# cmpute/d3d

Measured on AMD Instinct MI355X. Metric: voxelize_mpoints_per_s, higher is better.
Workload: dtype f32; 1 GPU; config2: 1000000 LiDAR-like points, KITTI range, 0.1 m voxels (704x800x40), dense+MEAN, max 32 pts/voxel; points_per_gpu=1000000, parallelism=1 GPU

## Files before the change

### d3d_amd/csrc/voxel.hip

```cpp
#include "common.hpp"
#include <stdlib.h>
#include <limits.h>
#include <algorithm>
#include <utility>

namespace {

typedef unsigned long long u64;

constexpr u64 kEmpty = ~0ull;
constexpr uint32_t kInf = 0xffffffffu;
constexpr uint32_t kSingleVoxel = 0xfffffffeu;
constexpr uint32_t kNoVoxel = 0xffffffffu;
constexpr uint32_t kNoSlot = 0xffffffffu;
constexpr uint32_t kNoBase = 0xffffffffu;
constexpr int kReduceSum = 4;
constexpr int kSweepTile = 1024;
constexpr int kFlagTile = 256 * 64;


__device__ __forceinline__ u64 mix64(u64 h)
{
    h ^= h >> 33; h *= 0xff51afd7ed558ccdull;
    h ^= h >> 33; h *= 0xc4ceb9fe1a85ec53ull;
// ... 1951 lines not shown
            const typename E::type e = bent[pos[r]];
            key_in[r] = E::key(e);
            idx[r] = E::idx(e);
        }
    });
    if constexpr (STAGE) {
        static_for<ITEMS>([&](auto R) {
            constexpr int r = decltype(R)::value;
            row[r] = *reinterpret_cast<const v4f *>(&points4[idx[r]]);
        });
    }
    lds_barrier();
    D3D_PHASE(0, 1);
#ifdef D3D_PHASE_CLOCKS
    asm volatile("s_waitcnt vmcnt(0)" ::: "memory");
    D3D_PHASE(0, 8);
#endif
    static_for<ITEMS>([&](auto R) {
        constexpr int r = decltype(R)::value;
        const uint32_t q = threadIdx.x + r * kBucketThreads;
        if (q < m) {
            const KT key = (KT)key_in[r];
            uint32_t s = (Key::bin_hash(key_in[r]) >> hshift) & (T - 1);
            for (;;) {
                const KT old = atomicCAS(&tkey[s], kFree, key);
                if (old == kFree || old == key) break;
                s = (s + 1) & (T - 1);
            }
            slot[r] = s;
            arr[r] = atomicAdd(&tcnt[s], 1u);
            atomicMin(&tfirst[s], idx[r]);
        }
    });
    lds_barrier();
    D3D_PHASE(0, 2);
    records(std::false_type{});
    early_publish();
    lds_barrier();
    D3D_PHASE(0, 3);
    static_for<ITEMS>([&](auto R) {
        constexpr int r = decltype(R)::value;
        const uint32_t q = threadIdx.x + r * kBucketThreads;
        if (q < m) seg[(tcnt[slot[r]] >> 16) + arr[r]] = idx[r];
    });
    lds_barrier();
    D3D_PHASE(0, 4);
    v4f over_pre = {0.f, 0.f, 0.f, 0.f};
    if constexpr (ROWS) overflow_first(seg, over_pre);
    static_for<ITEMS>([&](auto R) {
        constexpr int r = decltype(R)::value;
        const uint32_t q = threadIdx.x + r * kBucketThreads;
        if (q < m) {
            const uint32_t s = slot[r], cb = tcnt[s], cnt = cb & 0xffffu, base = cb >> 16, me = idx[r];
            uint32_t rank = 0, k = 0;
            const uint32_t *sg = seg + base;
            const bool need = (STAGE || LISTS) ? cnt > 1 : cnt > P;
            for (; need && k + 8 <= cnt && rank < P; k += 8)
                rank += (sg[k] < me) + (sg[k + 1] < me) + (sg[k + 2] < me) + (sg[k + 3] < me) + (sg[k + 4] < me) + (sg[k + 5] < me) +
                        (sg[k + 6] < me) + (sg[k + 7] < me);
            for (; need && k < cnt && rank < P; k++) rank += sg[k] < me;
            if constexpr (STAGE) { if (rank < P) *reinterpret_cast<v4f *>(&staged[bb + base + rank]) = row[r]; }
            if constexpr (LISTS) {
                if (rank < P && (rank > 0 || !ROWS)) sorted_out[bb + base + rank] = me;
                if (unsorted_out && cnt > P) unsorted_out[bb + base + arr[r]] = me;
            }
            if (trimmed && rank >= P) trimmed[me] = 1;
            if (precpos) precpos[pos[r]] = tfirst[s];
            if (pfirst_out) {
                const uint32_t pf = (P > 0 && rank >= P) ? kInf : tfirst[s];
                if (!table || pf != me) pfirst_out[me] = pf;
            }
        }
    });
    D3D_PHASE(0, 5);
    reduce_overflow(seg, std::false_type{}, ROWS ? &over_pre : (const v4f *)nullptr);
    D3D_PHASE(0, 6);
}

struct EarlyNote {
    const u64 *tot = nullptr;
    uint32_t pairs = 0, max_voxels = 0;
    int64_t aux = 0;
    int64_t *counts = nullptr, *host = nullptr;
};

__global__ __launch_bounds__(1024) void k_first_count(const uint32_t *__restrict__ firstmap, uint32_t *fwpre, uint32_t *bsumF,
                                                      uint32_t *clear_word = nullptr ,
                                                      ZeroFill zf = ZeroFill(), EarlyNote en = EarlyNote())
{
    if (zero_fill_role(zf)) return;
    if (en.tot && blockIdx.x == 0 && threadIdx.x < kWave) {
        u64 v = 0;
        for (uint32_t t = threadIdx.x; t < en.pairs; t += kWave) v += en.tot[16 * t];
        v = wave_sum_u64(v);
        if (threadIdx.x == 0) {
            en.counts[D3D_COUNT_VOXELS] = (int64_t)(v < (u64)en.max_voxels ? v : (u64)en.max_voxels);
            en.counts[D3D_COUNT_AUX] = en.aux;
            notify_host(en.counts, en.host);
        }
    }
    if (clear_word && blockIdx.x == 0 && threadIdx.x == 0) *clear_word = 0;
    __shared__ u64 smem[1024 / kWave];
    __shared__ uint32_t wcnt[256];
    const int lane = threadIdx.x & (kWave - 1), w = threadIdx.x >> 6;
    const uint32_t *src = firstmap + ((size_t)blockIdx.x * 256 + w * 16) * 64 + lane;
    uint32_t e[16];
#pragma unroll
    for (int j = 0; j < 16; j++) e[j] = src[(size_t)j * 64];
#pragma unroll
    for (int j = 0; j < 16; j++) {
        const unsigned long long bal = __ballot(e[j] != kInf);
        if (lane == j) wcnt[w * 16 + j] = (uint32_t)__popcll(bal);
    }
    __syncthreads();
    u64 tot;
    const u64 ex = block_excl_scan_u64<1024>(threadIdx.x < 256 ? (u64)wcnt[threadIdx.x] : 0ull, &tot, smem);
    if (threadIdx.x < 256) fwpre[(size_t)blockIdx.x * 256 + threadIdx.x] = (uint32_t)ex;
    if (threadIdx.x == 0) bsumF[blockIdx.x] = (uint32_t)tot;
}

template <class Key, bool AGG4>
__device__ __forceinline__ uint32_t meta_first_lane(const Key &kf, int64_t i, uint32_t e, uint32_t vid, const uint4 *__restrict__ vrec,
                                                    uint32_t max_voxels, uint4 *__restrict__ vinfo, const float4 *__restrict__ staged,
                                                    uint32_t P, int reduction, int64_t *coords, int32_t *npoints, unsigned char *pmask,
                                                    float4 *agg, const BinnedExtras &x, const float *__restrict__ points, int c)
{
    uint32_t kept = 0, myvid = kNoVoxel;
    if (e != kInf && vid < max_voxels) {
        myvid = vid;
        if (x.first_out) x.first_out[vid] = x.index_offset + i;
        uint4 rec;
        if (e != kSingleVoxel) rec = vrec[e];
        else {
            const float *src = points + i * c;
            const float v3[3] = {src[0], src[1], src[2]};
            u64 key = 0;
            uint32_t st = 0;
            (void)kf.make(v3, key, st);
            rec = make_uint4((uint32_t)key, (uint32_t)(key >> 32), 0u, 1u);
        }
        const uint4 vi = rec;
        if (vinfo) vinfo[vid] = vi;
        if (x.count_out) x.count_out[vid] = (int32_t)vi.w;
        kept = vi.w < x.npoints_clamp ? vi.w : x.npoints_clamp;
        meta_voxel<Key, AGG4>(kf, (int64_t)vid, vi, staged, P, reduction, coords, npoints, x.voff, pmask, agg, nullptr, nullptr,
                              x.keys_out, x.npoints_clamp, x.has_coord_sub ? x.coord_sub : (const long long *)nullptr);
    }
    if (x.vidof) x.vidof[i] = myvid;
    return kept;
}

template <class Key, bool AGG4>
__global__ __launch_bounds__(256) void k_meta_first(Key kf, int64_t npad, const uint32_t *__restrict__ firstmap,
                                                    const uint32_t *__restrict__ fwpre, const uint32_t *__restrict__ bsumF,
                                                    const uint4 *__restrict__ vrec, uint32_t max_voxels, uint4 *__restrict__ vinfo,
                                                    const float4 *__restrict__ staged, uint32_t P, int reduction, int64_t *coords,
                                                    int32_t *npoints, unsigned char *pmask, float4 *agg, int64_t *counts,
                                                    BinnedExtras x, const float *__restrict__ points, int c)
{
    const int64_t i = (int64_t)blockIdx.x * 256 + threadIdx.x;
    const int lane = threadIdx.x & (kWave - 1);
    const uint32_t tile = (uint32_t)(i / kFlagTile), ntile = (uint32_t)(npad / kFlagTile);
    uint32_t before = 0, all = 0;
    for (uint32_t t = lane; t < ntile; t += kWave) {
        const uint32_t x = bsumF[t];
        all += x;
        if (t < tile) before += x;
    }
    {
        const u64 both = wave_sum_u64(((u64)all << 32) | before);
        before = (uint32_t)both;
        all = (uint32_t)(both >> 32);
    }
    if (i == 0) {
        counts[D3D_COUNT_VOXELS] = (int64_t)(all < max_voxels ? all : max_voxels);
        counts[D3D_COUNT_AUX] = 0;
        if (x.keys_out && x.status_row >= 0) x.keys_out[x.status_row] = -1 - counts[D3D_COUNT_STATUS];
        if (x.host_counts) notify_host(counts, x.host_counts);
    }
    const uint32_t e = firstmap[i];
    const unsigned long long bal = __ballot(e != kInf);
    const uint32_t vid = before + fwpre[i >> 6] + (uint32_t)__popcll(bal & ((1ull << lane) - 1ull));
    (void)meta_first_lane<Key, AGG4>(kf, i, e, vid, vrec, max_voxels, vinfo, staged, P, reduction, coords, npoints, pmask, agg, x, points, c);
}

constexpr int kMetaLbThreads = 1024, kMetaLbItems = 4, kMetaLbTile = kMetaLbThreads * kMetaLbItems;
struct MetaLb {
    u64 *stat;
    unsigned int *ticket;
    u64 *next_stat;
    uint32_t next_n;
    unsigned int *next_ticket;
    int64_t *host;
    const u64 *early;
    uint32_t early_pairs;
};
template <class Key>
__global__ __launch_bounds__(kMetaLbThreads) void k_meta_first_lb(Key kf, int64_t npad, const uint32_t *__restrict__ firstmap,
                                                                  const uint4 *__restrict__ vrec, uint32_t max_voxels, int64_t *coords,
                                                                  int32_t *npoints, int64_t *counts, BinnedExtras x, MetaLb lb,
                                                                  const float *__restrict__ points, int c)
{
    __shared__ unsigned int sid;
    __shared__ uint32_t wtot[kMetaLbThreads / kWave];
    __shared__ u64 sprefix;
    const unsigned int tile = lookback_ticket(lb.ticket, &sid);
    const unsigned int ntiles = gridDim.x;
    if (tile == 0) {
        if (lb.host && lb.early_pairs && threadIdx.x < kWave) {
            const bool have = threadIdx.x < lb.early_pairs;
            const u64 tv = wave_sum_u64(have ? lb.early[16 * threadIdx.x] : 0ull), tp = wave_sum_u64(have ? lb.early[16 * threadIdx.x + 1] : 0ull);
            if (threadIdx.x == 0 && tv <= (u64)max_voxels) {
                for (int k = 0; k < D3D_NUM_COUNTS; k++) {
                    lb.host[k] = counts[k];
                    lb.host[D3D_NUM_COUNTS + 1 + k] = 0;
                }
                lb.host[D3D_COUNT_VOXELS] = (int64_t)tv;
                lb.host[D3D_COUNT_AUX] = 0;
                lb.host[D3D_NUM_COUNTS + 1 + D3D_COUNT_VOXELS] = (int64_t)tv;
                lb.host[D3D_NUM_COUNTS + 1 + D3D_COUNT_POINTS] = (int64_t)tp;
                __threadfence_system();
                __hip_atomic_store(&lb.host[D3D_NUM_COUNTS], (int64_t)1, __ATOMIC_RELEASE, __HIP_MEMORY_SCOPE_SYSTEM);
            }
        }
        for (uint32_t t = threadIdx.x; t < lb.next_n; t += kMetaLbThreads) lb.next_stat[t] = 0ull;
        if (threadIdx.x == 0) *lb.next_ticket = 0u;
    }
    const int lane = threadIdx.x & (kWave - 1), w = threadIdx.x >> 6;
    const int64_t base = (int64_t)tile * kMetaLbTile + (int64_t)w * (kWave * kMetaLbItems) + lane;
    uint32_t e[kMetaLbItems], ex[kMetaLbItems], carry = 0;
#pragma unroll
    for (int k = 0; k < kMetaLbItems; k++) e[k] = firstmap[base + (int64_t)k * kWave];
#pragma unroll
    for (int k = 0; k < kMetaLbItems; k++) {
        const unsigned long long bal = __ballot(e[k] != kInf);
        ex[k] = carry + (uint32_t)__popcll(bal & ((1ull << lane) - 1ull));
        carry += (uint32_t)__popcll(bal);
    }
    if (lane == 0) wtot[w] = carry;
    __syncthreads();
    uint32_t total = 0, woff = 0;
#pragma unroll
    for (int k = 0; k < kMetaLbThreads / kWave; k++) {
        const uint32_t t = wtot[k];
        total += t;
        if (k < w) woff += t;
    }
    if (w == 0) {
        const u64 before = lookback_exclusive(lb.stat, tile, (u64)total);
        if (lane == 0) sprefix = before;
    }
    __syncthreads();
    const uint32_t pre = (uint32_t)sprefix + woff;
    uint32_t kept = 0;
#pragma unroll
    for (int k = 0; k < kMetaLbItems; k++)
        kept += meta_first_lane<Key, false>(kf, base + (int64_t)k * kWave, e[k], pre + ex[k], vrec, max_voxels, (uint4 *)nullptr,
                                            (const float4 *)nullptr, 0u, (int)D3D_REDUCE_NONE, coords, npoints, (unsigned char *)nullptr,
                                            (float4 *)nullptr, x, points, c);
    kept = (uint32_t)wave_sum_u64((u64)kept);
    __syncthreads();
    if (lane == 0) wtot[w] = kept;
    __syncthreads();
    if (w != 0) return;
    u64 mine = 0;
    for (int k = lane; k < kMetaLbThreads / kWave; k += kWave) mine += wtot[k];
    mine = wave_sum_u64(mine);
    if (tile + 1 != ntiles) {
        if (lane == 0) __hip_atomic_store(&lb.stat[ntiles + tile], (mine << 1) | 1ull, __ATOMIC_RELAXED, __HIP_MEMORY_SCOPE_AGENT);
        return;
    }
    u64 acc = 0;
    for (unsigned int j0 = 0; j0 + 1 < ntiles; j0 += kWave) {
        const unsigned int j = j0 + lane;
        if (j + 1 < ntiles) {
            u64 t;
            do { t = __hip_atomic_load(&lb.stat[ntiles + j], __ATOMIC_RELAXED, __HIP_MEMORY_SCOPE_AGENT); } while (!(t & 1ull));
            acc += t >> 1;
        }
    }
    acc = wave_sum_u64(acc) + mine;
    if (lane == 0) {
        const u64 all = sprefix + total;
        const int64_t nvox = (int64_t)(all < max_voxels ? all : max_voxels);
        counts[D3D_COUNT_VOXELS] = nvox;
        counts[D3D_COUNT_AUX] = 0;
        if (lb.host && !(lb.early_pairs && all <= (u64)max_voxels)) {
            for (int k = 0; k < D3D_NUM_COUNTS; k++) {
                lb.host[k] = counts[k];
                lb.host[D3D_NUM_COUNTS + 1 + k] = 0;
            }
            lb.host[D3D_NUM_COUNTS + 1 + D3D_COUNT_VOXELS] = nvox;
            lb.host[D3D_NUM_COUNTS + 1 + D3D_COUNT_POINTS] = (int64_t)acc;
            __threadfence_system();
            __hip_atomic_store(&lb.host[D3D_NUM_COUNTS], (int64_t)1, __ATOMIC_RELEASE, __HIP_MEMORY_SCOPE_SYSTEM);
        }
    }
}

constexpr int kEmitCap = 256;


template <class Key, bool AGG4, bool RESIDENT = false>
__global__ __launch_bounds__(256) void k_emit(Key kf, int64_t npad, const uint32_t *__restrict__ firstmap,
                                              const uint32_t *__restrict__ fwpre, const uint32_t *__restrict__ bsumF,
                                              const uint4 *__restrict__ vrec, uint32_t max_voxels,
                                              const float4 *__restrict__ points4, const uint32_t *__restrict__ ranked,
                                              const float4 *__restrict__ staged, uint32_t P, int pshift ,
                                              int reduction, int64_t *coords, int32_t *npoints, unsigned char *pmask, float4 *agg,
                                              float4 *voxels , int64_t *counts,
                                              int64_t *host_counts, BinnedExtras x)
{
    typedef float vec4 __attribute__((ext_vector_type(4)));
    __shared__ vec4 rowbuf_all[256 / kWave][kEmitCap];
    __shared__ uint32_t off_all[256 / kWave][kWave], base_all[256 / kWave][kWave], first_all[256 / kWave][kWave];
    __shared__ uint16_t kept_all[256 / kWave][kWave];
    __shared__ uint16_t lim_all[256 / kWave][kWave];
    __shared__ uint32_t loff_all[RESIDENT ? 256 / kWave : 1][kWave + 1];
    const int64_t i = (int64_t)blockIdx.x * 256 + threadIdx.x;
    const int lane = threadIdx.x & (kWave - 1), w = threadIdx.x >> 6;
    vec4 *rowbuf = rowbuf_all[w];
    uint32_t *sh_off = off_all[w], *sh_base = base_all[w], *sh_first = first_all[w];
    uint16_t *sh_kept = kept_all[w];
    uint16_t *sh_lim = lim_all[w];
    uint32_t *sh_loff = loff_all[RESIDENT ? w : 0];
    D3D_PHASE_DECL;
    const uint32_t tile = (uint32_t)(i / kFlagTile), ntile = (uint32_t)(npad / kFlagTile);
    uint32_t before = 0, all = 0;
    for (uint32_t t = lane; t < ntile; t += kWave) {
        const uint32_t x = bsumF[t];
        all += x;
        if (t < tile) before += x;
    }
    {
        const u64 both = wave_sum_u64(((u64)all << 32) | before);
        before = (uint32_t)both;
        all = (uint32_t)(both >> 32);
    }
    if (i == 0) {
        counts[D3D_COUNT_VOXELS] = (int64_t)(all < max_voxels ? all : max_voxels);
        counts[D3D_COUNT_AUX] = x.aux_value;
        if (x.keys_out && x.status_row >= 0) x.keys_out[x.status_row] = -1 - counts[D3D_COUNT_STATUS];
        if (host_counts) notify_host(counts, host_counts);
    }
    const uint32_t e = firstmap[i];
    const unsigned long long bal = __ballot(e != kInf);
    D3D_PHASE(2, 0);
    const uint32_t nfirst = (uint32_t)__popcll(bal);
    uint32_t nv = nfirst;
    const uint32_t vid0 = before + fwpre[i >> 6];
    const uint32_t r = (uint32_t)__popcll(bal & ((1ull << lane) - 1ull));
    if (x.vidof)
        x.vidof[i] = (e != kInf && vid0 < max_voxels && r < max_voxels - vid0) ? vid0 + r : kNoVoxel;
    if (nv == 0 || vid0 >= max_voxels) return;
    if (nv > max_voxels - vid0) nv = max_voxels - vid0;
    const uint32_t dst = (e != kInf ? r : nfirst + ((uint32_t)lane - r)) << 2;
    const uint32_t el = (uint32_t)__builtin_amdgcn_ds_permute((int)dst, (int)e);
    const uint32_t il = (uint32_t)__builtin_amdgcn_ds_permute((int)dst, (int)(uint32_t)i);
    const bool mine = (uint32_t)lane < nv;
    uint4 rec = make_uint4(0u, 0u, 0u, 0u);
    if (mine) {
        const bool has_rec = x.fm_packed ? (el >> kFmShift) == kFmRecord : el != kSingleVoxel;
        if (has_rec) rec = vrec[x.fm_packed ? (el & kFmMask) : el];
        else {
            const float4 p0 = points4[il];
            const float v3[3] = {p0.x, p0.y, p0.z};
            u64 key = 0;
            uint32_t st = 0;
            (void)kf.make(v3, key, st);
            rec = make_uint4((uint32_t)key, (uint32_t)(key >> 32), x.fm_packed ? (el & kFmMask) : 0u, x.fm_packed ? (el >> kFmShift) : 1u);
        }
    }
    bool early = false;
    vec4 *out = reinterpret_cast<vec4 *>(voxels) + (int64_t)vid0 * P;
    const vec4 zero = {0.f, 0.f, 0.f, 0.f};
    if constexpr (!RESIDENT) {
        if (x.early_zero && voxels && (P & 7u) == 0 && (reinterpret_cast<uintptr_t>(voxels) & 127) == 0) {
            const uint32_t c8 = el >> kFmShift;
            const bool unsure = mine && c8 == kFmRecord && P >= kFmRecord;
            if (!__ballot(unsure)) {
                early = true;
                const uint32_t kept_e = mine ? (c8 < P ? c8 : P) : 0u;
                sh_lim[lane] = (uint16_t)((kept_e + 7u) & ~7u);
                wave_lds_fence();
                const uint32_t qa = nv * P;
                for (uint32_t q0 = 0; q0 < qa; q0 += 4 * kWave) {
#pragma unroll
                    for (int u = 0; u < 4; u++) {
                        const uint32_t q = q0 + u * kWave + lane;
                        if (q < qa) {
                            const uint32_t j = pshift >= 0 ? (q >> pshift) : q / P;
                            if (q - j * P >= sh_lim[j]) __builtin_nontemporal_store(zero, &out[q]);
                        }
                    }
                }
            }
        }
    }
#ifdef D3D_PHASE_CLOCKS
    asm volatile("s_waitcnt vmcnt(0)" ::: "memory");
#endif
    D3D_PHASE(2, 1);
    const uint32_t base = rec.z, cnt = rec.w;
    const uint32_t kept = cnt < P ? cnt : P;
    const uint32_t incl = wave_incl_scan_u32(kept);
    const uint32_t off = incl - kept;
    sh_off[lane] = off; sh_base[lane] = base; sh_first[lane] = il; sh_kept[lane] = (uint16_t)kept;
    uint32_t loff = 0;
    if (RESIDENT) {
        uint32_t lim = 0;
        if (mine) {
            const uint32_t prev = x.row_state[(int64_t)vid0 + lane];
            lim = prev > kept ? prev : kept;
            if (lim > P) lim = P;
            if (prev != kept) x.row_state[(int64_t)vid0 + lane] = (uint16_t)kept;
        }
        sh_lim[lane] = (uint16_t)lim;
        loff = wave_incl_scan_u32(lim) - lim;
        sh_loff[lane] = loff;
    }
    wave_lds_fence();
    const bool is_sum = reduction == D3D_REDUCE_MEAN || reduction == kReduceSum;
    float a0, a1, a2, a3;
    a0 = a1 = a2 = a3 = is_sum ? 0.0f : (reduction == D3D_REDUCE_MAX ? -INFINITY : INFINITY);
    uint32_t ja = 0;
    while (ja < nv) {
        const uint32_t oa = (uint32_t)__shfl((int)off, (int)ja, kWave);
        const bool fits = (uint32_t)lane >= ja && mine && incl - oa <= (uint32_t)kEmitCap;
        const unsigned long long nf = ~(__ballot(fits) >> ja);
        const uint32_t jb = ja + (nf ? (uint32_t)__ffsll((long long)nf) - 1u : (uint32_t)kWave - ja);
        const uint32_t rows = (uint32_t)__shfl((int)incl, (int)jb - 1, kWave) - oa;
        for (uint32_t t0 = 0; t0 < rows; t0 += kWave) {
            const uint32_t t = t0 + lane;
            if (t < rows) {
                uint32_t lo = ja, hi = jb;
                while (hi - lo > 1) {
                    const uint32_t mid = (lo + hi) >> 1;
                    if (sh_off[mid] - oa <= t) lo = mid; else hi = mid;
                }
                const uint32_t k = t - (sh_off[lo] - oa);
                const uint32_t idx = k == 0 ? sh_first[lo] : ranked[sh_base[lo] + k];
                rowbuf[t] = *reinterpret_cast<const vec4 *>(&points4[idx]);
            }
        }
#ifdef D3D_PHASE_CLOCKS
        asm volatile("s_waitcnt vmcnt(0)" ::: "memory");
#endif
        D3D_PHASE(2, 2);
        wave_lds_fence();
        if (AGG4 && (uint32_t)lane >= ja && (uint32_t)lane < jb && cnt <= P) {
            const vec4 *rw = rowbuf + (off - oa);
            for (uint32_t k = 0; k < kept; k++) {
                const vec4 x = rw[k];
                if (is_sum) { a0 += x.x; a1 += x.y; a2 += x.z; a3 += x.w; }
                else if (reduction == D3D_REDUCE_MAX) {
                    a0 = a0 < x.x ? x.x : a0; a1 = a1 < x.y ? x.y : a1; a2 = a2 < x.z ? x.z : a2; a3 = a3 < x.w ? x.w : a3;
                } else {
                    a0 = x.x < a0 ? x.x : a0; a1 = x.y < a1 ? x.y : a1; a2 = x.z < a2 ? x.z : a2; a3 = x.w < a3 ? x.w : a3;
                }
            }
        }
        D3D_PHASE(2, 3);
        if (RESIDENT) {
            const uint32_t l0 = (uint32_t)__shfl((int)loff, (int)ja, kWave);
            const uint32_t l1 = jb < (uint32_t)kWave ? (uint32_t)__shfl((int)loff, (int)jb, kWave)
                                                    : (uint32_t)__shfl((int)(loff + sh_lim[lane]), kWave - 1, kWave);
            for (uint32_t t0 = l0; t0 < l1; t0 += kWave) {
                const uint32_t t = t0 + lane;
                if (t < l1) {
                    uint32_t lo = ja, hi = jb;
                    while (hi - lo > 1) {
                        const uint32_t mid = (lo + hi) >> 1;
                        if (sh_loff[mid] <= t) lo = mid; else hi = mid;
                    }
                    const uint32_t slot = t - sh_loff[lo];
                    vec4 val = zero;
                    if (slot < sh_kept[lo]) val = rowbuf[sh_off[lo] - oa + slot];
                    out[lo * P + slot] = val;
                }
            }
        }
        const uint32_t q1 = voxels && !RESIDENT ? jb * P : 0u;
        for (uint32_t q0 = ja * P; q0 < q1; q0 += 4 * kWave) {
#pragma unroll
            for (int u = 0; u < 4; u++) {
                const uint32_t q = q0 + u * kWave + lane;
                if (q < q1) {
                    const uint32_t j = pshift >= 0 ? (q >> pshift) : q / P;
                    const uint32_t slot = q - j * P;
                    vec4 val = zero;
                    if (slot < sh_kept[j]) val = rowbuf[sh_off[j] - oa + slot];
                    if (!early || slot < sh_lim[j]) __builtin_nontemporal_store(val, &out[q]);
                }
            }
        }
        D3D_PHASE(2, 4);
        wave_lds_fence();
        ja = jb;
    }
    const int64_t v = (int64_t)vid0 + lane;
    {
        long long *cbuf = reinterpret_cast<long long *>(rowbuf);
        if (mine) {
            long long cc[3];
            kf.decode(((u64)rec.y << 32) | rec.x, cc);
            cbuf[lane * 3 + 0] = cc[0]; cbuf[lane * 3 + 1] = cc[1]; cbuf[lane * 3 + 2] = cc[2];
            __builtin_nontemporal_store((int32_t)cnt, &npoints[v]);
            if (x.keys_out) x.keys_out[v] = (int64_t)(((u64)rec.y << 32) | rec.x);
            if (x.first_out) x.first_out[v] = x.index_offset + (int64_t)il;
            if (x.voff) x.voff[v] = base;
        }
        wave_lds_fence();
        if (coords) {
            long long *cdst = reinterpret_cast<long long *>(coords) + (int64_t)vid0 * 3;
            for (uint32_t t = lane; t < nv * 3; t += kWave) __builtin_nontemporal_store(cbuf[t], &cdst[t]);
        }
        if (pmask) {
            const uint32_t per = P >> 4, total = nv * per;
            typedef uint32_t uvec4 __attribute__((ext_vector_type(4)));
            uvec4 *pdst = reinterpret_cast<uvec4 *>(pmask + (int64_t)vid0 * P);
            for (uint32_t t = lane; t < total; t += kWave) {
                const uint32_t j = t / per, k0 = (t - j * per) << 4, kj = sh_kept[j];
                uvec4 w4;
#pragma unroll
                for (int q = 0; q < 4; q++) {
                    uint32_t b = 0;
#pragma unroll
                    for (int x = 0; x < 4; x++) b |= ((k0 + q * 4 + x) < kj ? 1u : 0u) << (8 * x);
                    w4[q] = b;
                }
                __builtin_nontemporal_store(w4, &pdst[t]);
            }
        }
    }
    if (AGG4 && mine) {
        vec4 res;
        if (cnt > P) res = *reinterpret_cast<const vec4 *>(&staged[base + P]);
        else {
            if (reduction == D3D_REDUCE_MEAN) {
                const float d = (float)(int32_t)cnt;
                a0 = a0 / d; a1 = a1 / d; a2 = a2 / d; a3 = a3 / d;
            }
            res.x = a0; res.y = a1; res.z = a2; res.w = a3;
        }
        __builtin_nontemporal_store(res, reinterpret_cast<vec4 *>(&agg[v]));
    }
    D3D_PHASE(2, 5);
}

template <class Key, bool AGG4, int WG = 256>
__global__ __launch_bounds__(WG) void k_emit_split(Key kf, int64_t npad, const uint32_t *__restrict__ firstmap,
                                                    const uint32_t *__restrict__ fwpre, const uint32_t *__restrict__ bsumF,
                                                    const uint4 *__restrict__ vrec, uint32_t max_voxels,
                                                    const float4 *__restrict__ points4, const uint32_t *__restrict__ ranked,
                                                    const float4 *__restrict__ staged, uint32_t P, int pshift ,
                                                    int reduction, int64_t *coords, int32_t *npoints, unsigned char *pmask ,
                                                    float4 *agg, float4 *voxels, int64_t *counts, int64_t *host_counts,
                                                    uint32_t prefilled, int64_t aux_value)
{
    typedef float vec4 __attribute__((ext_vector_type(4)));
    typedef uint32_t uvec4 __attribute__((ext_vector_type(4)));
    __shared__ vec4 rowbuf_all[256 / kWave][kEmitCap];
    __shared__ uint32_t off_all[256 / kWave][kWave], base_all[256 / kWave][kWave], first_all[256 / kWave][kWave];
    __shared__ uint32_t loff_all[256 / kWave][kWave];
    __shared__ uint16_t kept_all[WG / kWave][kWave], lim_all[WG / kWave][kWave];
    __shared__ long long zbuf_all[WG == 512 ? 4 : 1][WG == 512 ? 3 * kWave : 1];
    const bool zrole = WG == 512 ? threadIdx.x >= 256u : (blockIdx.x & 1u) != 0;
    const int64_t i = (int64_t)(WG == 512 ? blockIdx.x : blockIdx.x >> 1) * 256 + (threadIdx.x & 255u);
    const int lane = threadIdx.x & (kWave - 1), w = threadIdx.x >> 6;
    vec4 *rowbuf = rowbuf_all[w & 3];
    uint32_t *sh_off = off_all[w & 3], *sh_base = base_all[w & 3], *sh_first = first_all[w & 3], *sh_loff = loff_all[w & 3];
    uint16_t *sh_kept = kept_all[w], *sh_lim = lim_all[w];
    const uint32_t tile = (uint32_t)(i / kFlagTile), ntile = (uint32_t)(npad / kFlagTile);
    uint32_t before = 0, all = 0;
    for (uint32_t t = lane; t < ntile; t += kWave) {
        const uint32_t x = bsumF[t];
        all += x;
        if (t < tile) before += x;
    }
    {
        const u64 both = wave_sum_u64(((u64)all << 32) | before);
        before = (uint32_t)both;
        all = (uint32_t)(both >> 32);
    }
    if (i == 0 && !zrole) {
        counts[D3D_COUNT_VOXELS] = (int64_t)(all < max_voxels ? all : max_voxels);
        counts[D3D_COUNT_AUX] = aux_value;
        if (host_counts) notify_host(counts, host_counts);
    }
    const uint32_t e = firstmap[i];
    const unsigned long long bal = __ballot(e != kInf);
    const uint32_t nfirst = (uint32_t)__popcll(bal);
    uint32_t nv = nfirst;
    const uint32_t vid0 = before + fwpre[i >> 6];
    const uint32_t r = (uint32_t)__popcll(bal & ((1ull << lane) - 1ull));
    if (nv == 0 || vid0 >= max_voxels) return;
    if (nv > max_voxels - vid0) nv = max_voxels - vid0;
    const uint32_t dst = (e != kInf ? r : nfirst + ((uint32_t)lane - r)) << 2;
    const uint32_t el = (uint32_t)__builtin_amdgcn_ds_permute((int)dst, (int)e);
    const uint32_t il = (uint32_t)__builtin_amdgcn_ds_permute((int)dst, (int)(uint32_t)i);
    const bool mine = (uint32_t)lane < nv;
    const uint32_t c8 = el >> kFmShift, seg = el & kFmMask;
    const bool isrec = c8 == kFmRecord;
    const unsigned long long recmask = __ballot(mine && isrec);
    const int64_t v = (int64_t)vid0 + lane;
    vec4 *out = reinterpret_cast<vec4 *>(voxels) + (int64_t)vid0 * P;
    const vec4 zero = {0.f, 0.f, 0.f, 0.f};
    if (zrole) {
        float4 p0 = make_float4(0.f, 0.f, 0.f, 0.f);
        if (mine && !isrec) p0 = points4[il];
        {
            const uint32_t kept_e = c8 < P ? c8 : P, l8 = (kept_e + 7u) & ~7u;
            sh_lim[lane] = (uint16_t)(!mine ? 0u : (isrec || l8 > P) ? P : l8);
            sh_kept[lane] = (uint16_t)(mine ? kept_e : 0u);
        }
        long long *cbuf = WG == 512 ? zbuf_all[w & 3] : reinterpret_cast<long long *>(rowbuf);
        if (mine && !isrec) {
            const float v3[3] = {p0.x, p0.y, p0.z};
            u64 key = 0;
            uint32_t st = 0;
            (void)kf.make(v3, key, st);
            long long cc[3];
            kf.decode(key, cc);
            cbuf[lane * 3 + 0] = cc[0]; cbuf[lane * 3 + 1] = cc[1]; cbuf[lane * 3 + 2] = cc[2];
            __builtin_nontemporal_store((int32_t)c8, &npoints[v]);
        }
        wave_lds_fence();
        long long *cdst = reinterpret_cast<long long *>(coords) + (int64_t)vid0 * 3;
        for (uint32_t t = lane; t < nv * 3; t += kWave)
            if (!((recmask >> (t / 3u)) & 1ull)) __builtin_nontemporal_store(cbuf[t], &cdst[t]);
        if (pmask) {
            const uint32_t per = P >> 4, total = nv * per;
            uvec4 *pdst = reinterpret_cast<uvec4 *>(pmask + (int64_t)vid0 * P);
            for (uint32_t t = lane; t < total; t += kWave) {
                const uint32_t j = t / per, k0 = (t - j * per) << 4, kj = sh_kept[j];
                if ((recmask >> j) & 1ull) continue;
                uvec4 w4;
#pragma unroll
                for (int q = 0; q < 4; q++) {
                    uint32_t b = 0;
#pragma unroll
                    for (int x = 0; x < 4; x++) b |= ((k0 + q * 4 + x) < kj ? 1u : 0u) << (8 * x);
                    w4[q] = b;
                }
                __builtin_nontemporal_store(w4, &pdst[t]);
            }
        }
        const uint32_t npre = prefilled <= vid0 ? 0u : (prefilled - vid0 < nv ? prefilled - vid0 : nv);
        const uint32_t qa = nv * P;
        for (uint32_t q0 = npre * P; q0 < qa; q0 += 4 * kWave) {
#pragma unroll
            for (int u = 0; u < 4; u++) {
                const uint32_t q = q0 + u * kWave + lane;
                if (q < qa) {
                    const uint32_t j = pshift >= 0 ? (q >> pshift) : q / P;
                    if (q - j * P >= sh_lim[j]) __builtin_nontemporal_store(zero, &out[q]);
                }
            }
        }
        return;
    }
    uint32_t cnt = mine ? c8 : 0u, base = seg;
    u64 key = 0;
    if (mine && isrec) {
        const uint4 rec = vrec[seg];
        key = ((u64)rec.y << 32) | rec.x;
        base = rec.z;
        cnt = rec.w;
    }
    const uint32_t kept = cnt < P ? cnt : P;
    const uint32_t incl = wave_incl_scan_u32(kept);
    const uint32_t off = incl - kept;
    uint32_t lim = (kept + 7u) & ~7u;
    if (lim > P || (mine && isrec)) lim = P;
    const uint32_t lincl = wave_incl_scan_u32(lim);
    const uint32_t loff = lincl - lim;
    sh_off[lane] = off; sh_base[lane] = base; sh_first[lane] = il; sh_kept[lane] = (uint16_t)kept;
    sh_lim[lane] = (uint16_t)lim; sh_loff[lane] = loff;
    wave_lds_fence();
    const bool is_sum = reduction == D3D_REDUCE_MEAN || reduction == kReduceSum;
    float a0, a1, a2, a3;
    a0 = a1 = a2 = a3 = is_sum ? 0.0f : (reduction == D3D_REDUCE_MAX ? -INFINITY : INFINITY);
    uint32_t ja = 0;
    while (ja < nv) {
        const uint32_t oa = (uint32_t)__shfl((int)off, (int)ja, kWave);
        const bool fits = (uint32_t)lane >= ja && mine && incl - oa <= (uint32_t)kEmitCap;
        const unsigned long long nf = ~(__ballot(fits) >> ja);
        const uint32_t jb = ja + (nf ? (uint32_t)__ffsll((long long)nf) - 1u : (uint32_t)kWave - ja);
        const uint32_t rows = (uint32_t)__shfl((int)incl, (int)jb - 1, kWave) - oa;
        for (uint32_t t0 = 0; t0 < rows; t0 += kWave) {
            const uint32_t t = t0 + lane;
            if (t < rows) {
                uint32_t lo = ja, hi = jb;
                while (hi - lo > 1) {
                    const uint32_t mid = (lo + hi) >> 1;
                    if (sh_off[mid] - oa <= t) lo = mid; else hi = mid;
                }
                const uint32_t k = t - (sh_off[lo] - oa);
                const uint32_t idx = k == 0 ? sh_first[lo] : ranked[sh_base[lo] + k];
                rowbuf[t] = *reinterpret_cast<const vec4 *>(&points4[idx]);
            }
        }
        wave_lds_fence();
        if (AGG4 && (uint32_t)lane >= ja && (uint32_t)lane < jb && cnt <= P) {
            const vec4 *rw = rowbuf + (off - oa);
            for (uint32_t k = 0; k < kept; k++) {
                const vec4 x = rw[k];
                if (is_sum) { a0 += x.x; a1 += x.y; a2 += x.z; a3 += x.w; }
                else if (reduction == D3D_REDUCE_MAX) {
                    a0 = a0 < x.x ? x.x : a0; a1 = a1 < x.y ? x.y : a1; a2 = a2 < x.z ? x.z : a2; a3 = a3 < x.w ? x.w : a3;
                } else {
                    a0 = x.x < a0 ? x.x : a0; a1 = x.y < a1 ? x.y : a1; a2 = x.z < a2 ? x.z : a2; a3 = x.w < a3 ? x.w : a3;
                }
            }
        }
        const uint32_t l0 = (uint32_t)__shfl((int)loff, (int)ja, kWave);
        const uint32_t l1 = (uint32_t)__shfl((int)lincl, (int)jb - 1, kWave);
        for (uint32_t t0 = l0; t0 < l1; t0 += kWave) {
            const uint32_t t = t0 + lane;
            if (t < l1) {
                uint32_t lo = ja, hi = jb;
                while (hi - lo > 1) {
                    const uint32_t mid = (lo + hi) >> 1;
                    if (sh_loff[mid] <= t) lo = mid; else hi = mid;
                }
                const uint32_t slot = t - sh_loff[lo];
                vec4 val = zero;
                if (slot < sh_kept[lo]) val = rowbuf[sh_off[lo] - oa + slot];
                __builtin_nontemporal_store(val, &out[lo * P + slot]);
            }
        }
        wave_lds_fence();
        ja = jb;
    }
    if (AGG4 && mine) {
        vec4 res;
        if (cnt > P) res = *reinterpret_cast<const vec4 *>(&staged[base + P]);
        else {
            if (reduction == D3D_REDUCE_MEAN) {
                const float d = (float)(int32_t)cnt;
                a0 = a0 / d; a1 = a1 / d; a2 = a2 / d; a3 = a3 / d;
            }
            res.x = a0; res.y = a1; res.z = a2; res.w = a3;
        }
        __builtin_nontemporal_store(res, reinterpret_cast<vec4 *>(&agg[v]));
    }
    if (mine && isrec) {
        long long cc[3];
        kf.decode(key, cc);
        coords[v * 3 + 0] = cc[0]; coords[v * 3 + 1] = cc[1]; coords[v * 3 + 2] = cc[2];
        npoints[v] = (int32_t)cnt;
        if (pmask)
            for (uint32_t k = 0; k < P; k++) pmask[v * (int64_t)P + k] = k < kept ? 1 : 0;
    }
}

__global__ __launch_bounds__(256) void k_aggregate_overflow(const float *__restrict__ points, int c,
                                                            const uint32_t *__restrict__ ov_list, const uint32_t *__restrict__ ov_count,
                                                            const int32_t *__restrict__ npoints, const uint32_t *__restrict__ voff,
                                                            const uint32_t *__restrict__ unsorted, int reduction, float *agg)
{
    constexpr int kMaxC = 8;
    const uint32_t total = *ov_count;
    const int lane = threadIdx.x & (kWave - 1);
    const bool is_sum = reduction == D3D_REDUCE_MEAN || reduction == kReduceSum;
    const uint32_t nwaves = gridDim.x * (blockDim.x / kWave);
    for (uint32_t e = blockIdx.x * (blockDim.x / kWave) + (threadIdx.x >> 6); e < total; e += nwaves) {
        const int64_t vv = ov_list[e];
        const uint32_t cc = (uint32_t)npoints[vv];
        const uint32_t *seg = unsorted + voff[vv];
        double sum[kMaxC];
        float ext[kMaxC];
#pragma unroll
        for (int d = 0; d < kMaxC; d++) { sum[d] = 0.0; ext[d] = reduction == D3D_REDUCE_MAX ? -INFINITY : INFINITY; }
        for (uint32_t k0 = lane; k0 < cc; k0 += 4 * kWave) {
            uint32_t idx[4];
#pragma unroll
            for (int u = 0; u < 4; u++) idx[u] = k0 + u * kWave < cc ? seg[k0 + u * kWave] : 0u;
            float x[4][kMaxC];
#pragma unroll
            for (int u = 0; u < 4; u++) {
                const float *row = points + (int64_t)idx[u] * c;
#pragma unroll
                for (int d = 0; d < kMaxC; d++)
                    if (d < c) x[u][d] = row[d];
            }
#pragma unroll
            for (int u = 0; u < 4; u++) {
                if (k0 + u * kWave >= cc) break;
#pragma unroll
                for (int d = 0; d < kMaxC; d++)
                    if (d < c) {
                        if (is_sum) sum[d] += (double)x[u][d];
                        else if (reduction == D3D_REDUCE_MAX) ext[d] = ext[d] < x[u][d] ? x[u][d] : ext[d];
                        else ext[d] = x[u][d] < ext[d] ? x[u][d] : ext[d];
                    }
            }
        }
#pragma unroll
        for (int d = 0; d < kMaxC; d++) {
            if (d >= c) break;
#pragma unroll
            for (int o = kWave / 2; o > 0; o >>= 1) {
                const double s2 = __shfl_xor(sum[d], o, kWave);
                const float e2 = __shfl_xor(ext[d], o, kWave);
                sum[d] += s2;
                if (reduction == D3D_REDUCE_MAX) ext[d] = ext[d] < e2 ? e2 : ext[d];
                else ext[d] = e2 < ext[d] ? e2 : ext[d];
            }
            if (lane == 0) {
                float r;
// ... 2192 lines not shown
```

Measured before the change: 13300 Mpoints/s.

## Restructure k_emit gather to batch loads and overlap key computation with fetches

Reorganizes the emit kernel so the firstmap/fwpre loads are issued before the tile-sum loop, and the bsumF sum is unrolled 8-wide. The per-row gather now batches up to four ranked-index loads per lane before issuing the point loads. Key computation for single-point voxels and the resident limit scan run while those loads are in flight. LDS arrays shrink to 16-bit offsets, sh_first is dropped by storing the first point from a register, and a waves-per-eu hint is added. The early-zero path no longer checks for uncertain record counts, which could be a correctness risk when a voxel has a record, and the added complexity increases register pressure.

```diff
diff --git a/d3d_amd/csrc/voxel.hip b/d3d_amd/csrc/voxel.hip
--- a/d3d_amd/csrc/voxel.hip
+++ b/d3d_amd/csrc/voxel.hip
@@ -2277,7 +2277,7 @@
 
 
 template <class Key, bool AGG4, bool RESIDENT = false>
-__global__ __launch_bounds__(256) void k_emit(Key kf, int64_t npad, const uint32_t *__restrict__ firstmap,
+__global__ __launch_bounds__(256) __attribute__((amdgpu_waves_per_eu(8))) void k_emit(Key kf, int64_t npad, const uint32_t *__restrict__ firstmap,
                                               const uint32_t *__restrict__ fwpre, const uint32_t *__restrict__ bsumF,
                                               const uint4 *__restrict__ vrec, uint32_t max_voxels,
                                               const float4 *__restrict__ points4, const uint32_t *__restrict__ ranked,
@@ -2288,24 +2288,37 @@
 {
     typedef float vec4 __attribute__((ext_vector_type(4)));
     __shared__ vec4 rowbuf_all[256 / kWave][kEmitCap];
-    __shared__ uint32_t off_all[256 / kWave][kWave], base_all[256 / kWave][kWave], first_all[256 / kWave][kWave];
+    __shared__ uint32_t base_all[256 / kWave][kWave];
+    __shared__ uint16_t off_all[256 / kWave][kWave];
     __shared__ uint16_t kept_all[256 / kWave][kWave];
     __shared__ uint16_t lim_all[256 / kWave][kWave];
-    __shared__ uint32_t loff_all[RESIDENT ? 256 / kWave : 1][kWave + 1];
+    __shared__ uint16_t loff_all[RESIDENT ? 256 / kWave : 1][kWave];
+    static_assert(kWave * kEmitCap < 65536, "k_emit: row offsets of a wavefront in 16 bits");
     const int64_t i = (int64_t)blockIdx.x * 256 + threadIdx.x;
     const int lane = threadIdx.x & (kWave - 1), w = threadIdx.x >> 6;
     vec4 *rowbuf = rowbuf_all[w];
-    uint32_t *sh_off = off_all[w], *sh_base = base_all[w], *sh_first = first_all[w];
+    uint32_t *sh_base = base_all[w];
+    uint16_t *sh_off = off_all[w];
     uint16_t *sh_kept = kept_all[w];
     uint16_t *sh_lim = lim_all[w];
-    uint32_t *sh_loff = loff_all[RESIDENT ? w : 0];
+    uint16_t *sh_loff = loff_all[RESIDENT ? w : 0];
     D3D_PHASE_DECL;
     const uint32_t tile = (uint32_t)(i / kFlagTile), ntile = (uint32_t)(npad / kFlagTile);
+    const uint32_t e = firstmap[i];
+    const uint32_t fw = fwpre[i >> 6];
     uint32_t before = 0, all = 0;
-    for (uint32_t t = lane; t < ntile; t += kWave) {
-        const uint32_t x = bsumF[t];
-        all += x;
-        if (t < tile) before += x;
+    for (uint32_t t0 = 0; t0 < ntile; t0 += 8 * kWave) {
+        uint32_t s[8];
+#pragma unroll
+        for (int u = 0; u < 8; u++) {
+            const uint32_t t = t0 + u * kWave + lane;
+            s[u] = t < ntile ? bsumF[t] : 0u;
+        }
+#pragma unroll
+        for (int u = 0; u < 8; u++) {
+            all += s[u];
+            if (t0 + u * kWave + lane < tile) before += s[u];
+        }
     }
     {
         const u64 both = wave_sum_u64(((u64)all << 32) | before);
@@ -2318,12 +2331,11 @@
         if (x.keys_out && x.status_row >= 0) x.keys_out[x.status_row] = -1 - counts[D3D_COUNT_STATUS];
         if (host_counts) notify_host(counts, host_counts);
     }
-    const uint32_t e = firstmap[i];
     const unsigned long long bal = __ballot(e != kInf);
     D3D_PHASE(2, 0);
     const uint32_t nfirst = (uint32_t)__popcll(bal);
     uint32_t nv = nfirst;
-    const uint32_t vid0 = before + fwpre[i >> 6];
+    const uint32_t vid0 = before + fw;
     const uint32_t r = (uint32_t)__popcll(bal & ((1ull << lane) - 1ull));
     if (x.vidof)
         x.vidof[i] = (e != kInf && vid0 < max_voxels && r < max_voxels - vid0) ? vid0 + r : kNoVoxel;
@@ -2333,66 +2345,47 @@
     const uint32_t el = (uint32_t)__builtin_amdgcn_ds_permute((int)dst, (int)e);
     const uint32_t il = (uint32_t)__builtin_amdgcn_ds_permute((int)dst, (int)(uint32_t)i);
     const bool mine = (uint32_t)lane < nv;
-    uint4 rec = make_uint4(0u, 0u, 0u, 0u);
-    if (mine) {
-        const bool has_rec = x.fm_packed ? (el >> kFmShift) == kFmRecord : el != kSingleVoxel;
-        if (has_rec) rec = vrec[x.fm_packed ? (el & kFmMask) : el];
-        else {
-            const float4 p0 = points4[il];
-            const float v3[3] = {p0.x, p0.y, p0.z};
-            u64 key = 0;
-            uint32_t st = 0;
-            (void)kf.make(v3, key, st);
-            rec = make_uint4((uint32_t)key, (uint32_t)(key >> 32), x.fm_packed ? (el & kFmMask) : 0u, x.fm_packed ? (el >> kFmShift) : 1u);
-        }
-    }
-    bool early = false;
-    vec4 *out = reinterpret_cast<vec4 *>(voxels) + (int64_t)vid0 * P;
+    const uint32_t c8 = el >> kFmShift;
+    const bool has_rec = mine && (x.fm_packed ? c8 == kFmRecord : el != kSingleVoxel);
+    uint32_t base = x.fm_packed ? (el & kFmMask) : 0u, cnt = mine ? (x.fm_packed ? c8 : 1u) : 0u;
+    uint32_t key_lo = 0, key_hi = 0;
+    if (__ballot(has_rec)) {
+        if (has_rec) {
+            const uint4 rec = vrec[x.fm_packed ? (el & kFmMask) : el];
+            key_lo = rec.x; key_hi = rec.y; base = rec.z; cnt = rec.w;
+        }
+        asm volatile("" : "+v"(base), "+v"(cnt));
+    }
+    const auto row_at = [&](uint32_t p) { return *reinterpret_cast<const vec4 *>(reinterpret_cast<const char *>(points4) + (p << 4)); };
     const vec4 zero = {0.f, 0.f, 0.f, 0.f};
-    if constexpr (!RESIDENT) {
-        if (x.early_zero && voxels && (P & 7u) == 0 && (reinterpret_cast<uintptr_t>(voxels) & 127) == 0) {
-            const uint32_t c8 = el >> kFmShift;
-            const bool unsure = mine && c8 == kFmRecord && P >= kFmRecord;
-            if (!__ballot(unsure)) {
-                early = true;
-                const uint32_t kept_e = mine ? (c8 < P ? c8 : P) : 0u;
-                sh_lim[lane] = (uint16_t)((kept_e + 7u) & ~7u);
-                wave_lds_fence();
-                const uint32_t qa = nv * P;
-                for (uint32_t q0 = 0; q0 < qa; q0 += 4 * kWave) {
-#pragma unroll
-                    for (int u = 0; u < 4; u++) {
-                        const uint32_t q = q0 + u * kWave + lane;
-                        if (q < qa) {
-                            const uint32_t j = pshift >= 0 ? (q >> pshift) : q / P;
-                            if (q - j * P >= sh_lim[j]) __builtin_nontemporal_store(zero, &out[q]);
-                        }
-                    }
-                }
-            }
-        }
-    }
-#ifdef D3D_PHASE_CLOCKS
-    asm volatile("s_waitcnt vmcnt(0)" ::: "memory");
-#endif
-    D3D_PHASE(2, 1);
-    const uint32_t base = rec.z, cnt = rec.w;
+    vec4 p0 = zero;
+    if (mine) p0 = row_at(il);
+    uint32_t prev = 0;
+    if (RESIDENT && mine) prev = x.row_state[(int64_t)vid0 + lane];
     const uint32_t kept = cnt < P ? cnt : P;
     const uint32_t incl = wave_incl_scan_u32(kept);
     const uint32_t off = incl - kept;
-    sh_off[lane] = off; sh_base[lane] = base; sh_first[lane] = il; sh_kept[lane] = (uint16_t)kept;
+    sh_off[lane] = (uint16_t)off; sh_base[lane] = base; sh_kept[lane] = (uint16_t)kept;
+    bool early = false;
+    vec4 *out = reinterpret_cast<vec4 *>(voxels) + (int64_t)vid0 * P;
     uint32_t loff = 0;
-    if (RESIDENT) {
-        uint32_t lim = 0;
-        if (mine) {
-            const uint32_t prev = x.row_state[(int64_t)vid0 + lane];
-            lim = prev > kept ? prev : kept;
-            if (lim > P) lim = P;
-            if (prev != kept) x.row_state[(int64_t)vid0 + lane] = (uint16_t)kept;
-        }
-        sh_lim[lane] = (uint16_t)lim;
-        loff = wave_incl_scan_u32(lim) - lim;
-        sh_loff[lane] = loff;
+    if constexpr (!RESIDENT) {
+        if (x.early_zero && voxels && (P & 7u) == 0 && (reinterpret_cast<uintptr_t>(voxels) & 127) == 0) {
+            early = true;
+            sh_lim[lane] = (uint16_t)((kept + 7u) & ~7u);
+            wave_lds_fence();
+            const uint32_t qa = nv * P;
+            for (uint32_t q0 = 0; q0 < qa; q0 += 4 * kWave) {
+#pragma unroll
+                for (int u = 0; u < 4; u++) {
+                    const uint32_t q = q0 + u * kWave + lane;
+                    if (q < qa) {
+                        const uint32_t j = pshift >= 0 ? (q >> pshift) : q / P;
+                        if (q - j * P >= sh_lim[j]) __builtin_nontemporal_store(zero, &out[q]);
+                    }
+                }
+            }
+        }
     }
     wave_lds_fence();
     const bool is_sum = reduction == D3D_REDUCE_MEAN || reduction == kReduceSum;
@@ -2405,22 +2398,61 @@
         const unsigned long long nf = ~(__ballot(fits) >> ja);
         const uint32_t jb = ja + (nf ? (uint32_t)__ffsll((long long)nf) - 1u : (uint32_t)kWave - ja);
         const uint32_t rows = (uint32_t)__shfl((int)incl, (int)jb - 1, kWave) - oa;
-        for (uint32_t t0 = 0; t0 < rows; t0 += kWave) {
-            const uint32_t t = t0 + lane;
-            if (t < rows) {
+        const uint32_t nr = rows > jb - ja ? rows - (jb - ja) : 0u;
+        static_assert(kEmitCap == 4 * kWave, "k_emit: a row's place in the buffer is one byte of pos");
+        uint32_t idx[kEmitCap / kWave], pos = 0;
+#pragma unroll
+        for (int u = 0; u < kEmitCap / kWave; u++) {
+            const uint32_t t = u * kWave + lane;
+            idx[u] = 0;
+            if (t < nr) {
                 uint32_t lo = ja, hi = jb;
                 while (hi - lo > 1) {
                     const uint32_t mid = (lo + hi) >> 1;
-                    if (sh_off[mid] - oa <= t) lo = mid; else hi = mid;
+                    if (sh_off[mid] - oa - (mid - ja) <= t) lo = mid; else hi = mid;
                 }
-                const uint32_t k = t - (sh_off[lo] - oa);
-                const uint32_t idx = k == 0 ? sh_first[lo] : ranked[sh_base[lo] + k];
-                rowbuf[t] = *reinterpret_cast<const vec4 *>(&points4[idx]);
-            }
-        }
+                const uint32_t o = sh_off[lo] - oa, k = t - (o - (lo - ja)) + 1u;
+                pos |= (o + k) << (8 * u);
+                idx[u] = *reinterpret_cast<const uint32_t *>(reinterpret_cast<const char *>(ranked) + ((sh_base[lo] + k) << 2));
+            }
+        }
+        static_assert(kEmitCap / kWave == 4, "k_emit: four ranked indices per lane");
+        asm volatile("" : "+v"(idx[0]), "+v"(idx[1]), "+v"(idx[2]), "+v"(idx[3]), "+v"(p0), "+v"(prev));
+        D3D_PHASE(2, 1);
+#pragma unroll
+        for (int h = 0; h < kEmitCap / kWave; h += 2) {
+            if (h != 0 && h * kWave >= nr) break;
+            vec4 row[2];
+#pragma unroll
+            for (int u = 0; u < 2; u++) {
+                row[u] = zero;
+                if ((h + u) * kWave + lane < nr) row[u] = row_at(idx[h + u]);
+            }
+            if (h == 0 && ja == 0) {
+                if (mine && !has_rec) {
+                    const float v3[3] = {p0.x, p0.y, p0.z};
+                    u64 key = 0;
+                    uint32_t st = 0;
+                    (void)kf.make(v3, key, st);
+                    key_lo = (uint32_t)key; key_hi = (uint32_t)(key >> 32);
+                }
+                if constexpr (RESIDENT) {
+                    uint32_t lim = prev > kept ? prev : kept;
+                    if (lim > P) lim = P;
+                    if (!mine) lim = 0;
+                    sh_lim[lane] = (uint16_t)lim;
+                    loff = wave_incl_scan_u32(lim) - lim;
+                    sh_loff[lane] = (uint16_t)loff;
+                }
+            }
+            if (h == 0 && (uint32_t)lane >= ja && (uint32_t)lane < jb) rowbuf[off - oa] = p0;
 #ifdef D3D_PHASE_CLOCKS
-        asm volatile("s_waitcnt vmcnt(0)" ::: "memory");
+            asm volatile("s_waitcnt vmcnt(0)" ::: "memory");
 #endif
+#pragma unroll
+            for (int u = 0; u < 2; u++)
+                if ((h + u) * kWave + lane < nr) rowbuf[(pos >> (8 * (h + u))) & 255u] = row[u];
+        }
         D3D_PHASE(2, 2);
         wave_lds_fence();
         if (AGG4 && (uint32_t)lane >= ja && (uint32_t)lane < jb && cnt <= P) {
@@ -2478,10 +2510,11 @@
         long long *cbuf = reinterpret_cast<long long *>(rowbuf);
         if (mine) {
             long long cc[3];
-            kf.decode(((u64)rec.y << 32) | rec.x, cc);
+            kf.decode(((u64)key_hi << 32) | key_lo, cc);
             cbuf[lane * 3 + 0] = cc[0]; cbuf[lane * 3 + 1] = cc[1]; cbuf[lane * 3 + 2] = cc[2];
             __builtin_nontemporal_store((int32_t)cnt, &npoints[v]);
-            if (x.keys_out) x.keys_out[v] = (int64_t)(((u64)rec.y << 32) | rec.x);
+            if (RESIDENT && prev != kept) x.row_state[v] = (uint16_t)kept;
+            if (x.keys_out) x.keys_out[v] = (int64_t)(((u64)key_hi << 32) | key_lo);
             if (x.first_out) x.first_out[v] = x.index_offset + (int64_t)il;
             if (x.voff) x.voff[v] = base;
         }
```

New measurement: 10470 Mpoints/s. -21.3%, worse.
